# facebookresearch/VideoPose3D

Measured on NVIDIA H100. Metric: frames/sec (arc 3,3,3,3,3, T=243, N=1024), higher is better.
Workload: dtype fp16 (IEEE fp16 operands and activations, fp32 accumulate)

## Files before the change

videopose3d_b200/csrc/api.cu:

```cuda
#include <cuda.h>
#include <cuda_runtime.h>
#include <stdarg.h>
#include <stdio.h>
#include <stdlib.h>
#include <string.h>

#include <string>
#include <vector>

#include "internal.cuh"
#include "pack.cuh"
#include "train_ops.cuh"

using namespace vp3d;

static thread_local char g_err[512] = "";
namespace vp3d {
int fail(int code, const char* fmt, ...) {
  va_list ap;
  va_start(ap, fmt);
  vsnprintf(g_err, sizeof(g_err), fmt, ap);
  va_end(ap);
  return code;
}
// ... 57 lines not shown
                   box, estr, CU_TENSOR_MAP_INTERLEAVE_NONE, CU_TENSOR_MAP_SWIZZLE_128B,
                   CU_TENSOR_MAP_L2_PROMOTION_L2_256B, CU_TENSOR_MAP_FLOAT_OOB_FILL_NONE);
  if (r != CUDA_SUCCESS)
    return fail(VP3D_ERR_CUDA, "cuTensorMapEncodeTiled(2d) failed: %d (inner=%llu rows=%llu)",
                (int)r, (unsigned long long)inner, (unsigned long long)rows);
  return VP3D_OK;
}

int pick_block_n(int n_pad) {
  if (n_pad % 128 == 0) return 128;
  return 64;
}

static int g_sm_limit = 0;
int num_sms() {
  static int cache[kMaxDevices] = {};
  int dev = 0;
  if (cudaGetDevice(&dev) != cudaSuccess || dev < 0 || dev >= kMaxDevices) return 132;
  if (!cache[dev]) {
    int n = 0;
    cudaDeviceGetAttribute(&n, cudaDevAttrMultiProcessorCount, dev);
    cache[dev] = n > 0 ? n : 132;
    if (const char* e = getenv("VP3D_SM_LIMIT")) {
      const int lim = atoi(e);
      if (lim >= 2 && !g_sm_limit) g_sm_limit = lim;
    }
  }
  int n = cache[dev];
  if (g_sm_limit >= 2 && g_sm_limit < n) n = g_sm_limit;
  return n;
}

struct ConvLaunch {
  CUtensorMap ma, mw, mo, mr, mz;
  ConvGemmArgs g;
  int block_n = 64;
  int sms = 0;
  bool empty = false;
};

static int prepare_conv(const vp3d_conv_desc* d, ConvLaunch* L) {
  if (!d || !d->a || !d->w) return fail(VP3D_ERR_INVALID, "conv_gemm: null operand");
  if (d->a_ld % 64 || d->k_per_tap % 64 || d->n_pad % 64)
    return fail(VP3D_ERR_INVALID, "conv_gemm: a_ld, k_per_tap and n_pad must be multiples of 64");
  if (d->taps < 1 || d->out_rows < 0 || d->samples < 1)
    return fail(VP3D_ERR_INVALID, "conv_gemm: bad geometry");
  L->empty = d->out_rows == 0;
  if (L->empty) return VP3D_OK;
  const int a_planes = d->a_planes > 0 ? d->a_planes : 1;
  const int pairs = d->precision == VP3D_PRECISION_BF16X3 ? 3 : 1;
  const int i8 = d->precision == VP3D_PRECISION_INT8 ? 1 : 0;
  const int f16 = (d->precision == VP3D_PRECISION_FP16 || i8) ? 1 : 0;
  if (f16 && (a_planes != 1 || d->out_planes > 1 || d->stats || d->bnb_z))
    return fail(VP3D_ERR_INVALID, "conv_gemm: fp16 is a single-plane, inference-only format");
  if (i8 && (d->k_per_tap % kBlockK8 || d->tap_col_step != 0))
    return fail(VP3D_ERR_INVALID, "conv_gemm: int8 needs k_per_tap %% 128 == 0 and taps that step "
                "rows (tap_col_step 0)");
  if (d->out_u8 && (!f16 || d->out_u8_ld % 16 || d->out_u8_ld < d->n_pad ||
                    reinterpret_cast<uintptr_t>(d->out_u8) % 16))
    return fail(VP3D_ERR_INVALID, "conv_gemm: a u8 output needs fp16 or int8, a 16-byte aligned "
                "pointer and out_u8_ld >= n_pad, a multiple of 16");
  if ((i8 || d->out_u8) &&
      (!d->scale || !d->shift || !d->relu || d->out_f32 || d->res_col_begin || d->res_cols ||
       (d->res && d->res_planes > 1) || (i8 && d->res && !d->out) ||
       (i8 && !d->res && (d->out || !d->out_u8)) || (!i8 && (!d->out || d->res))))
    return fail(VP3D_ERR_UNSUPPORTED, "conv_gemm: int8 and u8 outputs exist for affine + ReLU "
                "[+ one-plane residual over every column] launches: int8 writes u8 alone or, with a "
// ... 110 lines not shown
      g.res_tma_col_off = (int)col_off;
      g.res_tma_row_off = (int)row_off;
    }
  }
  CUtensorMap& mz = L->mz;
  mz = mo;
  g.bnb = 0;
  if (d->bnb_z) {
    if (!d->out || g.out_planes != 1 || (d->res && !g.res_tma) || d->bnb_c <= 0 || d->bnb_c % 64)
      return fail(VP3D_ERR_INVALID, "conv_gemm: fused BN-backward needs a single-plane bf16 output, "
                  "a TMA-loadable residual (if any) and bnb_c % 64 == 0");
    const uint64_t o_rows = d->out_rows, o_ld = d->out_ld;
    const uint64_t o_samples = d->per_sample_tiles ? d->samples : 1;
    VP3D_TRY(make_map_4d(&mz, d->bnb_z, o_ld, o_rows, o_ld, o_samples, o_rows * o_ld, 1,
                         o_samples * o_rows * o_ld, kBlockM));
    g.bnb = 1;
    g.bnb_c = d->bnb_c;
    g.bnb_scale = d->bnb_scale; g.bnb_shift = d->bnb_shift; g.bnb_mean = d->bnb_mean;
    g.bnb_invstd = d->bnb_invstd; g.bnb_sums = d->bnb_sums;
    g.bnb_p = d->bnb_p;
    g.bnb_seed_lo = (unsigned)(d->bnb_seed & 0xFFFFFFFFu);
    g.bnb_seed_hi = (unsigned)(d->bnb_seed >> 32);
    g.bnb_layer = (unsigned)d->bnb_layer;
  }
  if (d->out_u8) {
    const uint64_t rows = d->out_rows, ld = d->out_u8_ld;
    const uint64_t smp = d->per_sample_tiles ? d->samples : 1;
    VP3D_TRY(make_map_4d(&mz, d->out_u8, d->n_pad, rows, ld, smp, rows * ld, 1, smp * rows * ld, 32,
                         1, 64, CU_TENSOR_MAP_SWIZZLE_NONE));
  }
  if ((i8 || d->out_u8) && d->res && !g.res_tma)
    return fail(VP3D_ERR_UNSUPPORTED, "conv_gemm: int8 / u8-output launches need a residual that "
                "TMA can load (one box of a strided row view)");
  VP3D_TRY(make_map_2d(&mw, d->w, d->k_per_tap, (uint64_t)w_planes * d->taps * d->n_pad, block_n,
                       i8 ? 1 : 2));
  return VP3D_OK;
}

int run_conv(const vp3d_conv_desc* d, cudaStream_t stream) {
  ConvLaunch L;
  VP3D_TRY(prepare_conv(d, &L));
  if (L.empty) return VP3D_OK;
  CUDA_TRY(launch_conv_gemm(L.ma, L.mw, L.mo, L.mr, L.mz, L.g, L.block_n, L.sms, stream));
  return VP3D_OK;
}

static int conv_instance(const vp3d_conv_desc* d, int* key) {
  if (!key) return fail(VP3D_ERR_INVALID, "conv_gemm_instance: null key");
  ConvLaunch L;
  VP3D_TRY(prepare_conv(d, &L));
  if (L.empty) return fail(VP3D_ERR_INVALID, "conv_gemm_instance: no output rows, nothing is launched");
  if (!conv_gemm_instance(L.g, L.block_n, L.sms, key))
    return fail(VP3D_ERR_UNSUPPORTED, "conv_gemm_instance: the selected instance is not compiled");
  return VP3D_OK;
}

int plan_alloc(vp3d_plan* p, void** out, size_t bytes) {
  void* q = nullptr;
  CUDA_TRY(cudaMalloc(&q, bytes));
  p->allocs.push_back(q);
  *out = q;
  return VP3D_OK;
}

static int conv_k_pad(const vp3d_plan* p, int l) {
  return block_is_int8(p, l / 2 + 1) ? round_up(p->C, kBlockK8) : p->C;
}

static size_t pack_capacity(const vp3d_plan* p, const PackedConv& k) {
  const size_t b = pack_bytes(p, k);
  if (!p->int8 || k.transposed || k.src < 0) return b;
  const size_t b16 = (size_t)k.stored_taps * k.n_pad * p->C * sizeof(__nv_bfloat16);
  return b > b16 ? b : b16;
}

static void plan_packs(vp3d_plan* p) {
// ... 907 lines not shown
```

videopose3d_b200/csrc/conv_gemm.cu:

```cuda
#include "conv_gemm.cuh"

#include <stdlib.h>
#include <string.h>

#include <type_traits>

#include "ptx.cuh"

namespace vp3d {

enum class Epi { kTrain, kGeneral, kLean };
enum class Fmt { kRuntime, kBf16, kF16, kI8 };
enum class Sched { kCooperative, kPingPong };
enum class U8Out { kNone, kBeside, kAlone };

struct InstKey {
  int block_n;
  Epi epi;
  Fmt fmt;
  Sched sched;
  bool res;
  bool out2;
  U8Out u8;
  constexpr bool operator==(const InstKey& o) const {
// ... 35 lines not shown
  static constexpr uint32_t kHalfBytes = 64 * 64 * 2;
  static constexpr uint32_t kStagingBytes =
      kPP ? (RES ? 0 : 2 * kTileBytes) : 2 * 2 * (OUT2 ? 2 : 1) * kHalfBytes;
  static constexpr int kResSlots = RES ? 4 : 0;
  static constexpr uint32_t kU8Bytes = kU8Beside ? 2 * kBlockM * 64 : 0;
  static constexpr uint32_t kFixedBytes = kStagingBytes + kResSlots * kTileBytes + kU8Bytes;
  static constexpr uint32_t kAffineBytes = kPP ? 0 : 2 * BLOCK_N * 4;
  static constexpr uint32_t kPairBytes = kTrain ? 4 * 2 * 64 * 4 : 0;
  static constexpr uint32_t kBarBytesMax = (2 * 8 + 8 + 1) * 8 + 32;
  static constexpr uint32_t kMaxSmem = 232448u;
  static constexpr int kStagesFit =
      (kMaxSmem - 1024 - kFixedBytes - kBarBytesMax - kAffineBytes - kPairBytes) / kStageBytes;
  static constexpr int kStages = kStagesFit > 8 ? 8 : kStagesFit;
  static_assert(kStages >= 2, "not enough shared memory for the operand pipeline");
  static constexpr uint32_t kBarBytes = (2 * kStages + 8 + 1) * 8 + 32;
  static constexpr uint32_t kSmemBytes =
      1024 + kStages * kStageBytes + kFixedBytes + kBarBytes + kAffineBytes + kPairBytes;
  static_assert(kSmemBytes <= kMaxSmem, "shared memory budget exceeded");
};

__device__ __forceinline__ void tile_coords(const ConvGemmArgs& p, int tile, int& n_blk,
                                            int& sample, int& row0) {
  n_blk = tile % p.n_tiles;
  int m_blk = tile / p.n_tiles;
  if (p.dilated) {
    sample = m_blk / p.tiles_per_sample;
    row0 = (m_blk - sample * p.tiles_per_sample) * kBlockM;
  } else {
    sample = 0;
    row0 = m_blk * kBlockM;
  }
}

__device__ __forceinline__ uint32_t ld_shared_u32(uint32_t addr) {
  uint32_t v;
  asm volatile("ld.shared.b32 %0, [%1];" : "=r"(v) : "r"(addr) : "memory");
  return v;
}
__device__ __forceinline__ void st_shared_u32(uint32_t addr, uint32_t v) {
  asm volatile("st.shared.b32 [%0], %1;" ::"r"(addr), "r"(v) : "memory");
}
__device__ __forceinline__ uint32_t sw128_off(int row, int c) {
  return (uint32_t)row * 128u + ((((uint32_t)c >> 3) ^ ((uint32_t)row & 7u)) << 4) + ((uint32_t)c & 7u) * 2u;
}
__device__ __forceinline__ void add_pair(float& a, float& b, uint32_t u, bool f16) {
  if (f16) { a += f16_lo_to_f(u); b += f16_hi_to_f(u); }
  else { a += bf16_lo_to_f(u); b += bf16_hi_to_f(u); }
}

__device__ __forceinline__ void st_u8_pair(uint32_t addr, float v0, float v1, float inv_s) {
  const uint32_t q = quant_u8(v0, inv_s) | (quant_u8(v1, inv_s) << 8);
  asm volatile("st.shared.u16 [%0], %1;" ::"r"(addr), "h"((unsigned short)q) : "memory");
}

__device__ __forceinline__ void slab_reduce(float (&s)[8][2], float (&q)[8][2], float* s_pair,
                                            int lane, int wq, uint32_t bar_id) {
#pragma unroll
  for (int off = 4; off <= 16; off <<= 1) {
#pragma unroll
    for (int jj = 0; jj < 8; ++jj) {
#pragma unroll
      for (int e = 0; e < 2; ++e) {
        s[jj][e] += __shfl_xor_sync(0xffffffffu, s[jj][e], off);
        q[jj][e] += __shfl_xor_sync(0xffffffffu, q[jj][e], off);
      }
    }
// ... 5 lines not shown
      *reinterpret_cast<float2*>(s_pair + 64 + 8 * jj + 2 * lane) = make_float2(q[jj][0], q[jj][1]);
    }
  }
  named_bar_sync(bar_id, 64);
  if (!(wq & 1) && lane < 4) {
#pragma unroll
    for (int jj = 0; jj < 8; ++jj) {
      const float2 so = *reinterpret_cast<const float2*>(s_pair + 8 * jj + 2 * lane);
      const float2 qo = *reinterpret_cast<const float2*>(s_pair + 64 + 8 * jj + 2 * lane);
      s[jj][0] += so.x; s[jj][1] += so.y;
      q[jj][0] += qo.x; q[jj][1] += qo.y;
    }
  }
  named_bar_sync(bar_id, 64);
}

#ifdef VP3D_TIMELINE
__device__ __forceinline__ void tl_stamp(const ConvGemmArgs& p, int ev) {
  if (!p.timeline) return;
  int slot;
  if (blockIdx.x == 0) slot = 0;
  else if (blockIdx.x == gridDim.x - 1) slot = 1;
  else return;
  unsigned long long g;
  asm volatile("mov.u64 %0, %%globaltimer;" : "=l"(g));
  p.timeline[(slot * 32 + ev) * 2] = g;
  p.timeline[(slot * 32 + ev) * 2 + 1] = (unsigned long long)clock64();
}
#define TL(ev) tl_stamp(p, ev)
#else
#define TL(ev) ((void)0)
#endif

template <int BLOCK_N, Fmt FMT, int H, class Acc>
__device__ __forceinline__ void wgmma_kblock(Acc (&acc)[H][BLOCK_N / 2], const uint64_t (&da)[H],
                                             uint64_t db, bool first) {
#pragma unroll
  for (int h = 0; h < H; ++h) {
#pragma unroll
    for (int k = 0; k < 4; ++k) {
      const uint32_t accumulate = (first && k == 0) ? 0u : 1u;
      if constexpr (FMT == Fmt::kI8) {
        if constexpr (BLOCK_N == 128) wgmma_m64n128k32_u8s8(acc[h], da[h] + 2 * k, db + 2 * k, accumulate);
        else wgmma_m64n64k32_u8s8(acc[h], da[h] + 2 * k, db + 2 * k, accumulate);
      } else if constexpr (BLOCK_N == 128) {
        if constexpr (FMT == Fmt::kF16) wgmma_m64n128_f16(acc[h], da[h] + 2 * k, db + 2 * k, accumulate);
        else wgmma_m64n128_bf16(acc[h], da[h] + 2 * k, db + 2 * k, accumulate);
      } else {
        if constexpr (FMT == Fmt::kF16) wgmma_m64n64_f16(acc[h], da[h] + 2 * k, db + 2 * k, accumulate);
        else wgmma_m64n64_bf16(acc[h], da[h] + 2 * k, db + 2 * k, accumulate);
      }
    }
  }
}

template <class I, int H, class Issued>
__device__ __forceinline__ void mma_tile(typename I::Acc (&acc)[H][I::kBlockN / 2],
                                         const ConvGemmArgs& p, bool f16, uint32_t smem_a,
                                         uint32_t a_off, uint32_t smem_b, uint32_t full_bar,
                                         uint32_t empty_bar, uint32_t& stage_io, uint32_t& phase_io,
                                         int k_iters, int lane, bool tl_first, Issued issued) {
  uint32_t stage = stage_io, phase = phase_io;
  uint32_t prev_stage = 0;
  for (int it = 0; it < k_iters; ++it) {
    mbar_wait(full_bar + stage * 8, phase);
#ifdef VP3D_TIMELINE
    if (tl_first && it == 0) TL(4);
#endif
    const uint32_t a_st = smem_a + stage * I::kABytes + a_off;
    uint64_t da[H];
#pragma unroll
    for (int h = 0; h < H; ++h) da[h] = make_gmma_desc_sw128(a_st + h * 64 * 128, 16, 1024);
    const uint64_t db = make_gmma_desc_sw128(smem_b + stage * I::kBBytes, 16, 1024);
#pragma unroll
    for (int h = 0; h < H; ++h) wgmma_fence_operands(acc[h]);
    wgmma_fence();
    if constexpr (I::kFmt != Fmt::kRuntime) wgmma_kblock<I::kBlockN, I::kFmt>(acc, da, db, it == 0);
    else if (f16) wgmma_kblock<I::kBlockN, Fmt::kF16>(acc, da, db, it == 0);
    else wgmma_kblock<I::kBlockN, Fmt::kBf16>(acc, da, db, it == 0);
    wgmma_commit();
#pragma unroll
    for (int h = 0; h < H; ++h) wgmma_fence_operands(acc[h]);
    if (it > 0) {
      wgmma_wait<1>();
#pragma unroll
      for (int h = 0; h < H; ++h) wgmma_fence_operands(acc[h]);
      if (lane == 0) mbar_arrive(empty_bar + prev_stage * 8);
    }
    prev_stage = stage;
    if (++stage == I::kStages) { stage = 0; phase ^= 1; }
  }
  stage_io = stage; phase_io = phase;
  issued();
  wgmma_wait<0>();
#pragma unroll
  for (int h = 0; h < H; ++h) wgmma_fence_operands(acc[h]);
  if (k_iters > 0 && lane == 0) mbar_arrive(empty_bar + prev_stage * 8);
}

template <class I>
__global__ void __launch_bounds__(384, 1)
conv_gemm_kernel(const __grid_constant__ CUtensorMap tmap_a,
                 const __grid_constant__ CUtensorMap tmap_w,
                 const __grid_constant__ CUtensorMap tmap_out,
                 const __grid_constant__ CUtensorMap tmap_res,
                 const __grid_constant__ CUtensorMap tmap_z, const ConvGemmArgs p) {
  using Acc = typename I::Acc;
  constexpr int kBlocksPerTile = I::kBlockN / 64;
  constexpr int kFrag = I::kBlockN / 2;
  constexpr int kBK = I::kI8 ? kBlockK8 : kBlockK;

  extern __shared__ uint8_t smem_raw[];
  const uint32_t raw_addr = smem_u32(smem_raw);
  const uint32_t base = (raw_addr + 1023u) & ~1023u;
  uint8_t* smem = smem_raw + (base - raw_addr);

  const uint32_t smem_a = base;
  const uint32_t smem_b = base + I::kStages * I::kABytes;
  const uint32_t smem_store = base + I::kStages * I::kStageBytes;
  const uint32_t smem_res = smem_store + I::kStagingBytes;
  const uint32_t smem_u8 = smem_res + I::kResSlots * I::kTileBytes;
  const uint32_t bar_base = smem_u8 + I::kU8Bytes;
  const uint32_t full_bar = bar_base;
  const uint32_t empty_bar = bar_base + I::kStages * 8;
  const uint32_t rfull_bar = bar_base + 2 * I::kStages * 8;
  const uint32_t rempty_bar = rfull_bar + 32;
  const uint32_t dep_bar = rempty_bar + 32;
  const uint32_t affine_off = (dep_bar + 8 - base + 15u) & ~15u;
  float* s_affine = reinterpret_cast<float*>(smem + affine_off);
  float* s_pairs = reinterpret_cast<float*>(smem + affine_off + I::kAffineBytes);

  const int warp = threadIdx.x >> 5;
  const int lane = threadIdx.x & 31;
  if (threadIdx.x == 0) TL(0);

  const int m_tiles = p.dilated ? p.samples * p.tiles_per_sample : p.tiles_per_sample;
  const int total_tiles = m_tiles * p.n_tiles;
  const int k_iters = p.pairs * p.taps * p.kblocks_per_tap;
  const bool has_res = (p.flags & kEpiResidual) != 0;
  const bool bnb = I::kTrain && p.bnb != 0;
  const int aux_tiles = (has_res ? p.res_planes : 0) + (bnb ? 1 : 0);
  const int res_stages =
      (aux_tiles > 0 && I::kResSlots >= aux_tiles) ? I::kResSlots / aux_tiles : 1;

  if (warp == 0 && lane == 0) {
    tma_prefetch_desc(&tmap_a);
    tma_prefetch_desc(&tmap_w);
    tma_prefetch_desc(&tmap_out);
    if (I::kRes) tma_prefetch_desc(&tmap_res);
    if (I::kRes && bnb) tma_prefetch_desc(&tmap_z);
    if (I::kU8) tma_prefetch_desc(&tmap_z);
  }
  if (warp == 1 && lane == 0) {
    for (int s = 0; s < I::kStages; ++s) {
      mbar_init(full_bar + s * 8, 1);
      mbar_init(empty_bar + s * 8, I::kPP ? 4 : 8);
    }
    for (int s = 0; s < 4; ++s) {
      mbar_init(rfull_bar + s * 8, 1);
      mbar_init(rempty_bar + s * 8, I::kPP ? 1 : 256);
    }
    mbar_init(dep_bar, 1);
    fence_mbar_init();
  }
  __syncthreads();
  if (threadIdx.x == 0) TL(1);
  if (warp != 0) {
    griddep_wait();
    griddep_launch_dependents();
  }
  if (threadIdx.x == 32) {
    mbar_arrive(dep_bar);
    TL(2);
  }

  if (warp == 0) {
    if (lane == 0) {
      constexpr bool kEarlyW = !I::kTrain;
      if (!kEarlyW) mbar_wait(dep_bar, 0);
      const int n_pre = kEarlyW ? (k_iters < I::kStages ? k_iters : I::kStages) : 0;
      int mode = n_pre > 0 ? 0 : 2;
      if (kEarlyW && mode == 2) mbar_wait(dep_bar, 0);
      int w = blockIdx.x;
      if (w < total_tiles) {
        int n_blk, sample, row0;
        tile_coords(p, w, n_blk, sample, row0);
        uint32_t stage = 0, phase = 0;
        int it = 0, pair = 0, tap = 0, kb = 0;
        for (;;) {
          const int a_plane = (pair == 1) ? 1 : 0;
          const int w_plane = (pair == 2) ? 1 : 0;
          const uint32_t fb = full_bar + stage * 8;
          if (mode != 1) {
            mbar_wait(empty_bar + stage * 8, phase ^ 1);
            mbar_expect_tx(fb, I::kStageBytes);
            const int w_row = (w_plane * p.taps + tap) * p.n_pad + n_blk * I::kBlockN;
            tma_load_2d(&tmap_w, fb, smem_b + stage * I::kBBytes, kb * kBK, w_row);
          }
          if (mode != 0) {
            const int a_row = row0 + tap * p.tap_row_step;
            const int a_col = tap * p.tap_col_step + kb * kBK;
            tma_load_4d(&tmap_a, fb, smem_a + stage * I::kABytes, a_col, a_row, sample, a_plane);
#ifdef VP3D_TIMELINE
            if (w == (int)blockIdx.x && it == 0) TL(3);
#endif
          }
          if (++stage == I::kStages) { stage = 0; phase ^= 1; }
          ++it;
          if (++kb == p.kblocks_per_tap) {
            kb = 0;
            if (++tap == p.taps) { tap = 0; ++pair; }
          }
          if (mode == 0 && it == n_pre) {
            mbar_wait(dep_bar, 0);
            mode = 1;
            it = 0; pair = 0; tap = 0; kb = 0;
            stage = 0; phase = 0;
          } else if (mode == 1 && it == n_pre) {
            mode = 2;
          }
          if (it == k_iters) {
            w += gridDim.x;
            if (w >= total_tiles) break;
            tile_coords(p, w, n_blk, sample, row0);
            it = 0; pair = 0; tap = 0; kb = 0;
          }
        }
      }
    }
  } else if (warp == 1) {
    if (I::kPP && I::kRes && lane == 0) {
      uint32_t filled[2] = {0u, 0u};
      for (int j = 0, w = blockIdx.x; w < total_tiles; ++j, w += gridDim.x) {
        int n_blk, sample, row0;
        tile_coords(p, w, n_blk, sample, row0);
        const int g = j & 1;
        for (int sb = 0; sb < kBlocksPerTile; ++sb) {
          const uint32_t n = g ? filled[1] : filled[0];
          const uint32_t slot = 2u * g + (n & 1u);
          mbar_wait(rempty_bar + slot * 8, ((n >> 1) & 1u) ^ 1u);
          mbar_expect_tx(rfull_bar + slot * 8, I::kTileBytes);
          tma_load_4d(&tmap_res, rfull_bar + slot * 8, smem_res + slot * I::kTileBytes,
                      n_blk * I::kBlockN + sb * 64 + p.res_tma_col_off, row0 + p.res_tma_row_off,
                      sample, 0);
          if (g) ++filled[1];
          else ++filled[0];
        }
      }
    } else if (!I::kPP && I::kRes && lane == 0) {
      uint32_t rs = 0, rphase = 0;
      for (int w = blockIdx.x; w < total_tiles; w += gridDim.x) {
        int n_blk, sample, row0;
        tile_coords(p, w, n_blk, sample, row0);
        for (int sb = 0; sb < kBlocksPerTile; ++sb) {
          const int col = n_blk * I::kBlockN + sb * 64;
          const bool res_here = has_res && col >= p.res_col_begin && col < p.res_col_begin + p.res_cols;
          if (!res_here && !bnb) continue;
          const int n_res = res_here ? p.res_planes : 0;
          mbar_wait(rempty_bar + rs * 8, rphase ^ 1);
          mbar_expect_tx(rfull_bar + rs * 8, (n_res + (bnb ? 1 : 0)) * I::kTileBytes);
          const uint32_t slot0 = smem_res + rs * aux_tiles * I::kTileBytes;
          for (int pl = 0; pl < n_res; ++pl)
            tma_load_4d(&tmap_res, rfull_bar + rs * 8, slot0 + pl * I::kTileBytes,
                        col - p.res_col_begin + p.res_tma_col_off, row0 + p.res_tma_row_off, sample,
                        pl);
          if (bnb)
            tma_load_4d(&tmap_z, rfull_bar + rs * 8, slot0 + (aux_tiles - 1) * I::kTileBytes, col,
                        row0, sample, 0);
          if (++rs == (uint32_t)res_stages) { rs = 0; rphase ^= 1; }
        }
      }
    }
  } else if (I::kPP && warp >= 4) {
    const int wg = (warp - 4) >> 2;
    const int wq = warp & 3;
    const int tid = (int)threadIdx.x - 128 - 128 * wg;
    const int rl0 = 16 * wq + (lane >> 2);
    const int cq = 2 * (lane & 3);
    const uint32_t bar_wg = 2u + (uint32_t)wg;
    const uint32_t bar_mine = 8u + (uint32_t)wg, bar_other = 9u - (uint32_t)wg;
    const uint32_t staging = smem_store + wg * I::kTileBytes;
    uint32_t res_seen = 0;
    Acc acc[2][kFrag];
#pragma unroll
    for (int i = 0; i < kFrag; ++i) acc[0][i] = acc[1][i] = 0.0f;

    for (int j = wg, w = blockIdx.x + wg * gridDim.x; w < total_tiles; j += 2, w += 2 * gridDim.x) {
      int n_blk, sample, row0;
      tile_coords(p, w, n_blk, sample, row0);

      const uint32_t fill = (uint32_t)j * (uint32_t)k_iters;
      uint32_t stage = fill % I::kStages, phase = (fill / I::kStages) & 1u;
      if (j > 0) named_bar_sync(bar_mine, 256);
      mma_tile<I>(acc, p, I::kF16, smem_a, 0u, smem_b, full_bar, empty_bar, stage, phase, k_iters,
                  lane, warp == 4 && lane == 0 && w == (int)blockIdx.x, [&] {
                    if (w + (int)gridDim.x < total_tiles) named_bar_arrive(bar_other, 256);
                  });
#ifdef VP3D_TIMELINE
      if (warp == 4 && lane == 0) { if (w == (int)blockIdx.x) TL(7); TL(8); }
#endif

      const float* scale = p.scale + n_blk * I::kBlockN;
      const float* shift = p.shift + n_blk * I::kBlockN;
#pragma unroll
      for (int sb = 0; sb < kBlocksPerTile; ++sb) {
        const int cb = n_blk * I::kBlockN + sb * 64;
        uint32_t tile_smem;
        if constexpr (I::kRes) {
          const uint32_t slot = 2u * wg + (res_seen & 1u);
          mbar_wait(rfull_bar + slot * 8, (res_seen >> 1) & 1u);
          ++res_seen;
          tile_smem = smem_res + slot * I::kTileBytes;
          if constexpr (I::kU8) {
            if (tid == 0) tma_store_wait_read<0>();
            named_bar_sync(bar_wg, 128);
          }
        } else {
          if (tid == 0) tma_store_wait_read<0>();
          named_bar_sync(bar_wg, 128);
          tile_smem = staging;
        }
        const uint32_t u8_tile = I::kU8Alone ? staging : smem_u8 + (uint32_t)wg * (kBlockM * 64);
#pragma unroll
        for (int jj = 0; jj < 8; ++jj) {
          const int j4 = 4 * (sb * 8 + jj);
          const int cl = sb * 64 + jj * 8 + cq;
          const float2 sc = __ldg(reinterpret_cast<const float2*>(scale + cl));
          const float2 sh = __ldg(reinterpret_cast<const float2*>(shift + cl));
#pragma unroll
          for (int h2 = 0; h2 < 2; ++h2) {
#pragma unroll
            for (int h = 0; h < 2; ++h) {
              float v0 = fmaxf(fmaf(static_cast<float>(acc[h2][j4 + 2 * h]), sc.x, sh.x), 0.0f);
              float v1 = fmaxf(fmaf(static_cast<float>(acc[h2][j4 + 2 * h + 1]), sc.y, sh.y), 0.0f);
              const uint32_t off = sw128_off(64 * h2 + rl0 + 8 * h, jj * 8 + cq);
              if (I::kRes) add_pair(v0, v1, ld_shared_u32(tile_smem + off), I::kF16);
              if constexpr (I::kStore16)
                st_shared_u32(tile_smem + off, I::kF16 ? pack_f16x2(v0, v1) : pack_bf16x2(v0, v1));
              if constexpr (I::kU8)
                st_u8_pair(u8_tile + (uint32_t)(64 * h2 + rl0 + 8 * h) * 64u + jj * 8 + cq, v0, v1,
                           p.u8_inv_s);
            }
          }
        }
        fence_proxy_async_smem();
        named_bar_sync(bar_wg, 128);
        if (tid == 0) {
#pragma unroll
          for (int hb = 0; hb < 4; ++hb) {
            if constexpr (I::kStore16)
              tma_store_4d(&tmap_out, tile_smem + hb * 4096u, cb, row0 + 32 * hb, sample, 0);
            if constexpr (I::kU8)
              tma_store_4d(&tmap_z, u8_tile + hb * 2048u, cb, row0 + 32 * hb, sample, 0);
          }
          tma_store_commit();
        }
      }
      if (I::kRes && tid == 0) {
        tma_store_wait_read<0>();
#pragma unroll
        for (int sb = 0; sb < kBlocksPerTile; ++sb)
          mbar_arrive(rempty_bar + (2u * wg + ((res_seen - kBlocksPerTile + sb) & 1u)) * 8);
      }
#ifdef VP3D_TIMELINE
      if (warp == 4 && lane == 0) { if (w == (int)blockIdx.x) TL(9); TL(10); }
#endif
    }
    if (tid == 0) tma_store_wait_all<0>();
#ifdef VP3D_TIMELINE
    if (warp == 4 && lane == 0) TL(11);
#endif
  } else if (!I::kPP && warp >= 4) {
    const int wg = (warp - 4) >> 2;
    const int wq = warp & 3;
    const int tid = (int)threadIdx.x - 128 - 128 * wg;
    const int rl0 = 16 * wq + (lane >> 2);
    const int cq = 2 * (lane & 3);
    const uint32_t bar_wg = 2u + (uint32_t)wg;
    const uint32_t bar_slab = 4u + (uint32_t)(wg * 2 + (wq >> 1));
    float* s_pair = s_pairs + (wg * 2 + (wq >> 1)) * 128;
    const bool f16 = I::kLean ? I::kF16 : p.f16 != 0;
    const bool do_relu = I::kLean || (p.flags & kEpiRelu);
    const bool do_res = I::kLean ? I::kRes : (p.flags & kEpiResidual) != 0;
    const bool do_stats = I::kTrain && (p.flags & kEpiStats);
    const bool do_f32 = !I::kLean && (p.flags & kEpiOutF32);
    const bool do_affine = I::kLean || (p.flags & kEpiAffine);
    const bool two_planes = I::kOut2 && p.out_planes == 2;
    uint32_t stage = 0, phase = 0;
    uint32_t ablock = 0;
    uint32_t sbuf = 0;
    int aff_n_blk = -1;
    Acc acc[1][kFrag];
#pragma unroll
    for (int i = 0; i < kFrag; ++i) acc[0][i] = 0.0f;

    for (int w = blockIdx.x; w < total_tiles; w += gridDim.x) {
      int n_blk, sample, row0;
      tile_coords(p, w, n_blk, sample, row0);
      const int m_blk = w / p.n_tiles;
// ... 203 lines not shown
          }
          sbuf ^= 1u;
        }
      }
#ifdef VP3D_TIMELINE
      if (warp == 4 && lane == 0) { if (w == (int)blockIdx.x) TL(9); TL(10); }
#endif
    }
    if (tid == 0) tma_store_wait_all<0>();
#ifdef VP3D_TIMELINE
    if (warp == 4 && lane == 0) TL(11);
#endif
  }
}

static int g_pdl = -1;
static bool pdl_enabled() {
  if (g_pdl < 0) {
    const char* e = getenv("VP3D_PDL");
    g_pdl = (e && e[0] == '0') ? 0 : 1;
  }
  return g_pdl != 0;
}
void conv_gemm_set_pdl(int on) { g_pdl = on ? 1 : 0; }
bool conv_gemm_pdl_enabled() { return pdl_enabled(); }

static int conv_tiles(const ConvGemmArgs& a) {
  const int m_tiles = a.dilated ? a.samples * a.tiles_per_sample : a.tiles_per_sample;
  return m_tiles * a.n_tiles;
}

template <class I>
static cudaError_t launch_impl(const CUtensorMap& tmap_a, const CUtensorMap& tmap_w,
                               const CUtensorMap& tmap_out, const CUtensorMap& tmap_res,
                               const CUtensorMap& tmap_z, const ConvGemmArgs& args, int num_sms,
                               cudaStream_t stream) {
  auto kernel = conv_gemm_kernel<I>;
  static bool attr_set[kMaxDevices] = {};
  int dev = 0;
  cudaError_t e = cudaGetDevice(&dev);
  if (e != cudaSuccess) return e;
  if (dev < 0 || dev >= kMaxDevices) return cudaErrorInvalidDevice;
  if (!attr_set[dev]) {
    e = cudaFuncSetAttribute(kernel, cudaFuncAttributeMaxDynamicSharedMemorySize, I::kSmemBytes);
    if (e != cudaSuccess) return e;
    attr_set[dev] = true;
  }
  const int total = conv_tiles(args);
  if (total <= 0) return cudaSuccess;
  const int workers = total < num_sms ? total : num_sms;
  cudaLaunchConfig_t cfg;
  memset(&cfg, 0, sizeof(cfg));
  cfg.gridDim = dim3(workers, 1, 1);
  cfg.blockDim = dim3(384, 1, 1);
  cfg.dynamicSmemBytes = I::kSmemBytes;
  cfg.stream = stream;
  cudaLaunchAttribute attr[1];
  int n_attr = 0;
  if (pdl_enabled()) {
    attr[n_attr].id = cudaLaunchAttributeProgrammaticStreamSerialization;
    attr[n_attr].val.programmaticStreamSerializationAllowed = 1;
    ++n_attr;
  }
  cfg.attrs = attr;
  cfg.numAttrs = n_attr;
  return cudaLaunchKernelEx(&cfg, kernel, tmap_a, tmap_w, tmap_out, tmap_res, tmap_z, args);
}

static bool lean_enabled() {
  static int v = -1;
  if (v < 0) {
    const char* e = getenv("VP3D_LEAN");
    v = (e && e[0] == '0') ? 0 : 1;
  }
  return v != 0;
}
static bool lean_ok(const ConvGemmArgs& a, bool res) {
  if (!lean_enabled() || a.bnb || a.out_planes != 1 || !a.out) return false;
  if (!res) return a.flags == (kEpiAffine | kEpiRelu) && !a.res_tma;
  return a.flags == (kEpiAffine | kEpiRelu | kEpiResidual) && a.res_tma && a.res_planes == 1 &&
         a.res_col_begin == 0 && a.res_cols >= a.n_pad;
}

static InstKey select_instance(const ConvGemmArgs& a, int block_n, bool multi_tile) {
  InstKey k = {block_n, Epi::kGeneral, Fmt::kRuntime, Sched::kCooperative, a.res_tma || a.bnb,
               a.out_planes == 2 && !(a.flags & kEpiOutF32), U8Out::kNone};
  if ((a.flags & kEpiStats) || a.bnb) {
    k.epi = Epi::kTrain;
    return k;
  }
  const bool quant = a.i8 || a.out_u8;
  if (!quant && (k.out2 || !lean_ok(a, k.res))) return k;
  k.epi = Epi::kLean;
  k.fmt = a.i8 ? Fmt::kI8 : a.f16 ? Fmt::kF16 : Fmt::kBf16;
  if (a.out_u8) k.u8 = a.out ? U8Out::kBeside : U8Out::kAlone;
  if (multi_tile) k.sched = Sched::kPingPong;
  return k;
}

template <class... Is>
struct InstList {};

template <int BN>
using Instances = InstList<
    Inst<BN, Epi::kTrain, Fmt::kRuntime, Sched::kCooperative, false, false>,
    Inst<BN, Epi::kTrain, Fmt::kRuntime, Sched::kCooperative, false, true>,
    Inst<BN, Epi::kTrain, Fmt::kRuntime, Sched::kCooperative, true, false>,
    Inst<BN, Epi::kTrain, Fmt::kRuntime, Sched::kCooperative, true, true>,
    Inst<BN, Epi::kGeneral, Fmt::kRuntime, Sched::kCooperative, false, false>,
    Inst<BN, Epi::kGeneral, Fmt::kRuntime, Sched::kCooperative, false, true>,
    Inst<BN, Epi::kGeneral, Fmt::kRuntime, Sched::kCooperative, true, false>,
    Inst<BN, Epi::kGeneral, Fmt::kRuntime, Sched::kCooperative, true, true>,
    Inst<BN, Epi::kLean, Fmt::kBf16, Sched::kCooperative, false>,
    Inst<BN, Epi::kLean, Fmt::kBf16, Sched::kCooperative, true>,
    Inst<BN, Epi::kLean, Fmt::kBf16, Sched::kPingPong, false>,
    Inst<BN, Epi::kLean, Fmt::kBf16, Sched::kPingPong, true>,
    Inst<BN, Epi::kLean, Fmt::kF16, Sched::kCooperative, false>,
    Inst<BN, Epi::kLean, Fmt::kF16, Sched::kCooperative, true>,
    Inst<BN, Epi::kLean, Fmt::kF16, Sched::kPingPong, false>,
    Inst<BN, Epi::kLean, Fmt::kF16, Sched::kPingPong, true>,
    Inst<BN, Epi::kLean, Fmt::kI8, Sched::kCooperative, false, false, U8Out::kAlone>,
    Inst<BN, Epi::kLean, Fmt::kI8, Sched::kCooperative, true, false, U8Out::kNone>,
    Inst<BN, Epi::kLean, Fmt::kI8, Sched::kCooperative, true, false, U8Out::kBeside>,
    Inst<BN, Epi::kLean, Fmt::kF16, Sched::kCooperative, false, false, U8Out::kBeside>,
    Inst<BN, Epi::kLean, Fmt::kI8, Sched::kPingPong, false, false, U8Out::kAlone>,
    Inst<BN, Epi::kLean, Fmt::kI8, Sched::kPingPong, true, false, U8Out::kNone>,
    Inst<BN, Epi::kLean, Fmt::kI8, Sched::kPingPong, true, false, U8Out::kBeside>,
    Inst<BN, Epi::kLean, Fmt::kF16, Sched::kPingPong, false, false, U8Out::kBeside>>;

template <class... Is>
static cudaError_t launch_listed(InstList<Is...>, const InstKey& k, const CUtensorMap& a,
                                 const CUtensorMap& w, const CUtensorMap& o, const CUtensorMap& r,
                                 const CUtensorMap& z, const ConvGemmArgs& args, int num_sms,
                                 cudaStream_t stream) {
  cudaError_t e = cudaErrorInvalidValue;
  (void)((k == Is::kKey && ((e = launch_impl<Is>(a, w, o, r, z, args, num_sms, stream)), true)) ||
         ...);
  return e;
}

#ifdef VP3D_TIMELINE
static unsigned long long* g_timeline = nullptr;
static int g_timeline_max = 0, g_timeline_next = 0;
void conv_gemm_debug_set_timeline(unsigned long long* buf, int max_launches) {
  g_timeline = buf;
  g_timeline_max = max_launches;
  g_timeline_next = 0;
}
#endif

static InstKey launch_key(const ConvGemmArgs& args, int block_n, int num_sms) {
  return select_instance(args, block_n, conv_tiles(args) > num_sms);
}

template <class... Is>
static bool listed(InstList<Is...>, const InstKey& k) {
  return ((k == Is::kKey) || ...);
}

static void key_ints(const InstKey& k, int* out) {
  out[0] = k.block_n;
  out[1] = (int)k.epi;
  out[2] = (int)k.fmt;
  out[3] = (int)k.sched;
  out[4] = k.res ? 1 : 0;
  out[5] = k.out2 ? 1 : 0;
  out[6] = (int)k.u8;
}

bool conv_gemm_instance(const ConvGemmArgs& args, int block_n, int num_sms, int key[7]) {
  const InstKey k = launch_key(args, block_n, num_sms);
  key_ints(k, key);
  return block_n == 128 ? listed(Instances<128>{}, k) : listed(Instances<64>{}, k);
}

template <class... Is>
static int list_keys(InstList<Is...>, int* keys, int max) {
  const InstKey all[] = {Is::kKey...};
  const int n = (int)sizeof...(Is);
  for (int i = 0; i < n && i < max; ++i) key_ints(all[i], keys + 7 * i);
  return n;
}

int conv_gemm_instances(int* keys, int max) {
  const int n128 = list_keys(Instances<128>{}, keys, max);
  const int done = n128 < max ? n128 : max;
  return n128 + list_keys(Instances<64>{}, keys + 7 * done, max - done);
}

cudaError_t launch_conv_gemm(const CUtensorMap& tmap_a, const CUtensorMap& tmap_w,
                             const CUtensorMap& tmap_out, const CUtensorMap& tmap_res,
                             const CUtensorMap& tmap_z, const ConvGemmArgs& args_in, int block_n,
                             int num_sms, cudaStream_t stream) {
#ifdef VP3D_TIMELINE
  ConvGemmArgs args = args_in;
  args.timeline = (g_timeline && g_timeline_next < g_timeline_max)
                      ? g_timeline + (size_t)(g_timeline_next++) * 128 : nullptr;
#else
  const ConvGemmArgs& args = args_in;
#endif
  const InstKey k = launch_key(args, block_n, num_sms);
  if (block_n == 128)
    return launch_listed(Instances<128>{}, k, tmap_a, tmap_w, tmap_out, tmap_res, tmap_z, args, num_sms, stream);
  return launch_listed(Instances<64>{}, k, tmap_a, tmap_w, tmap_out, tmap_res, tmap_z, args, num_sms, stream);
}

}
```

videopose3d_b200/csrc/conv_gemm.cuh:

```cuda
#pragma once
#include <cuda.h>
#include <cuda_bf16.h>
#include <cuda_runtime.h>
#include <stdint.h>

namespace vp3d {

constexpr int kBlockM = 128;
constexpr int kBlockK = 64;
constexpr int kBlockK8 = 128;
constexpr int kUmmaK = 16;
constexpr int kMaxDevices = 64;

enum ConvGemmFlags : int {
  kEpiRelu = 1,
  kEpiResidual = 2,
  kEpiStats = 4,
  kEpiOutF32 = 8,
  kEpiAffine = 16,
};

struct ConvGemmArgs {
  int dilated;
  int samples;
// ... 15 lines not shown
  int res_planes;
  int res_ld;
  int res_rows_per_sample;
  int res_row_step;
  int res_row_off;
  int res_sample_div;
  int res_col_begin;
  int res_cols;
  int res_check_rows;
  int res_tma;
  int res_tma_col_off;
  int res_tma_row_off;
  int bnb;
  int bnb_c;
  const float* bnb_scale;
  const float* bnb_shift;
  const float* bnb_mean;
  const float* bnb_invstd;
  float* bnb_sums;
  float bnb_p;
  unsigned bnb_seed_lo, bnb_seed_hi, bnb_layer;
  __nv_bfloat16* out;
  long long out_plane_stride;
  int out_planes;
  int out_ld;
  float* out_f32;
  int out_f32_ld;
  int n_valid;
  float* stats;
  int lo_row_begin, lo_row_end;
  int i8;
  uint8_t* out_u8;
  float u8_inv_s;
#ifdef VP3D_TIMELINE
  unsigned long long* timeline;
#endif
};
#ifdef VP3D_TIMELINE
void conv_gemm_debug_set_timeline(unsigned long long* buf, int max_launches);
#endif

void conv_gemm_set_pdl(int on);
bool conv_gemm_pdl_enabled();
bool conv_gemm_instance(const ConvGemmArgs& args, int block_n, int num_sms, int key[7]);
int conv_gemm_instances(int* keys, int max);
cudaError_t launch_conv_gemm(const CUtensorMap& tmap_a, const CUtensorMap& tmap_w,
                             const CUtensorMap& tmap_out, const CUtensorMap& tmap_res,
                             const CUtensorMap& tmap_z, const ConvGemmArgs& args, int block_n,
                             int num_sms, cudaStream_t stream);

}
```

Measured before the change: 1.411 million.

## Split tail-wave 128-wide tiles into 64-wide halves in ping-pong conv GEMM

For ping-pong instances with 128-column tiles, the leftover tiles that would form a partial last wave are each split into two 64-column half items. These are spread across more CTAs using a separate 64-row weight tensor map and n64 wgmma. The aim is to shrink the wave-quantization tail, where only a few SMs are busy on the final tiles. The cost is extra A-tile loads for each half item and more complex producer, residual and epilogue bookkeeping.

```diff
diff --git a/videopose3d_b200/csrc/api.cu b/videopose3d_b200/csrc/api.cu
--- a/videopose3d_b200/csrc/api.cu
+++ b/videopose3d_b200/csrc/api.cu
@@ -113,7 +113,7 @@
 }
 
 struct ConvLaunch {
-  CUtensorMap ma, mw, mo, mr, mz;
+  CUtensorMap ma, mw, mw64, mo, mr, mz;
   ConvGemmArgs g;
   int block_n = 64;
   int sms = 0;
@@ -290,8 +290,10 @@
   if ((i8 || d->out_u8) && d->res && !g.res_tma)
     return fail(VP3D_ERR_UNSUPPORTED, "conv_gemm: int8 / u8-output launches need a residual that "
                 "TMA can load (one box of a strided row view)");
-  VP3D_TRY(make_map_2d(&mw, d->w, d->k_per_tap, (uint64_t)w_planes * d->taps * d->n_pad, block_n,
-                       i8 ? 1 : 2));
+  const uint64_t w_rows = (uint64_t)w_planes * d->taps * d->n_pad;
+  VP3D_TRY(make_map_2d(&mw, d->w, d->k_per_tap, w_rows, block_n, i8 ? 1 : 2));
+  L->mw64 = mw;
+  if (block_n == 128) VP3D_TRY(make_map_2d(&L->mw64, d->w, d->k_per_tap, w_rows, 64, i8 ? 1 : 2));
   return VP3D_OK;
 }
 
@@ -299,7 +301,7 @@
   ConvLaunch L;
   VP3D_TRY(prepare_conv(d, &L));
   if (L.empty) return VP3D_OK;
-  CUDA_TRY(launch_conv_gemm(L.ma, L.mw, L.mo, L.mr, L.mz, L.g, L.block_n, L.sms, stream));
+  CUDA_TRY(launch_conv_gemm(L.ma, L.mw, L.mw64, L.mo, L.mr, L.mz, L.g, L.block_n, L.sms, stream));
   return VP3D_OK;
 }
 
diff --git a/videopose3d_b200/csrc/conv_gemm.cu b/videopose3d_b200/csrc/conv_gemm.cu
--- a/videopose3d_b200/csrc/conv_gemm.cu
+++ b/videopose3d_b200/csrc/conv_gemm.cu
@@ -91,6 +91,14 @@
   }
 }
 
+__device__ __forceinline__ bool item_coords(const ConvGemmArgs& p, int full_tiles, int w,
+                                            int& n_blk, int& sample, int& row0, int& c_off) {
+  const bool half = w >= full_tiles;
+  c_off = half ? 64 * ((w - full_tiles) & 1) : 0;
+  tile_coords(p, half ? full_tiles + ((w - full_tiles) >> 1) : w, n_blk, sample, row0);
+  return half;
+}
+
 __device__ __forceinline__ uint32_t ld_shared_u32(uint32_t addr) {
   uint32_t v;
   asm volatile("ld.shared.b32 %0, [%1];" : "=r"(v) : "r"(addr) : "memory");
@@ -162,29 +170,31 @@
 #define TL(ev) ((void)0)
 #endif
 
-template <int BLOCK_N, Fmt FMT, int H, class Acc>
-__device__ __forceinline__ void wgmma_kblock(Acc (&acc)[H][BLOCK_N / 2], const uint64_t (&da)[H],
+template <int N, Fmt FMT, int H, int F, class Acc>
+__device__ __forceinline__ void wgmma_kblock(Acc (&acc)[H][F], const uint64_t (&da)[H],
                                              uint64_t db, bool first) {
+  static_assert((N == 64 || N == 128) && N / 2 <= F, "not a wgmma width of this accumulator");
 #pragma unroll
   for (int h = 0; h < H; ++h) {
+    auto& d = reinterpret_cast<Acc(&)[N / 2]>(acc[h]);
 #pragma unroll
     for (int k = 0; k < 4; ++k) {
       const uint32_t accumulate = (first && k == 0) ? 0u : 1u;
       if constexpr (FMT == Fmt::kI8) {
-        if constexpr (BLOCK_N == 128) wgmma_m64n128k32_u8s8(acc[h], da[h] + 2 * k, db + 2 * k, accumulate);
-        else wgmma_m64n64k32_u8s8(acc[h], da[h] + 2 * k, db + 2 * k, accumulate);
-      } else if constexpr (BLOCK_N == 128) {
-        if constexpr (FMT == Fmt::kF16) wgmma_m64n128_f16(acc[h], da[h] + 2 * k, db + 2 * k, accumulate);
-        else wgmma_m64n128_bf16(acc[h], da[h] + 2 * k, db + 2 * k, accumulate);
+        if constexpr (N == 128) wgmma_m64n128k32_u8s8(d, da[h] + 2 * k, db + 2 * k, accumulate);
+        else wgmma_m64n64k32_u8s8(d, da[h] + 2 * k, db + 2 * k, accumulate);
+      } else if constexpr (N == 128) {
+        if constexpr (FMT == Fmt::kF16) wgmma_m64n128_f16(d, da[h] + 2 * k, db + 2 * k, accumulate);
+        else wgmma_m64n128_bf16(d, da[h] + 2 * k, db + 2 * k, accumulate);
       } else {
-        if constexpr (FMT == Fmt::kF16) wgmma_m64n64_f16(acc[h], da[h] + 2 * k, db + 2 * k, accumulate);
-        else wgmma_m64n64_bf16(acc[h], da[h] + 2 * k, db + 2 * k, accumulate);
+        if constexpr (FMT == Fmt::kF16) wgmma_m64n64_f16(d, da[h] + 2 * k, db + 2 * k, accumulate);
+        else wgmma_m64n64_bf16(d, da[h] + 2 * k, db + 2 * k, accumulate);
       }
     }
   }
 }
 
-template <class I, int H, class Issued>
+template <class I, int N = I::kBlockN, int H, class Issued>
 __device__ __forceinline__ void mma_tile(typename I::Acc (&acc)[H][I::kBlockN / 2],
                                          const ConvGemmArgs& p, bool f16, uint32_t smem_a,
                                          uint32_t a_off, uint32_t smem_b, uint32_t full_bar,
@@ -205,9 +215,9 @@
 #pragma unroll
     for (int h = 0; h < H; ++h) wgmma_fence_operands(acc[h]);
     wgmma_fence();
-    if constexpr (I::kFmt != Fmt::kRuntime) wgmma_kblock<I::kBlockN, I::kFmt>(acc, da, db, it == 0);
-    else if (f16) wgmma_kblock<I::kBlockN, Fmt::kF16>(acc, da, db, it == 0);
-    else wgmma_kblock<I::kBlockN, Fmt::kBf16>(acc, da, db, it == 0);
+    if constexpr (I::kFmt != Fmt::kRuntime) wgmma_kblock<N, I::kFmt>(acc, da, db, it == 0);
+    else if (f16) wgmma_kblock<N, Fmt::kF16>(acc, da, db, it == 0);
+    else wgmma_kblock<N, Fmt::kBf16>(acc, da, db, it == 0);
     wgmma_commit();
 #pragma unroll
     for (int h = 0; h < H; ++h) wgmma_fence_operands(acc[h]);
@@ -232,6 +242,7 @@
 __global__ void __launch_bounds__(384, 1)
 conv_gemm_kernel(const __grid_constant__ CUtensorMap tmap_a,
                  const __grid_constant__ CUtensorMap tmap_w,
+                 const __grid_constant__ CUtensorMap tmap_w64,
                  const __grid_constant__ CUtensorMap tmap_out,
                  const __grid_constant__ CUtensorMap tmap_res,
                  const __grid_constant__ CUtensorMap tmap_z, const ConvGemmArgs p) {
@@ -266,6 +277,10 @@
 
   const int m_tiles = p.dilated ? p.samples * p.tiles_per_sample : p.tiles_per_sample;
   const int total_tiles = m_tiles * p.n_tiles;
+  constexpr bool kHalves = I::kPP && I::kBlockN == 128;
+  const int half_items = kHalves ? p.half_items : 0;
+  const int full_tiles = total_tiles - half_items / 2;
+  const int n_items = full_tiles + half_items;
   const int k_iters = p.pairs * p.taps * p.kblocks_per_tap;
   const bool has_res = (p.flags & kEpiResidual) != 0;
   const bool bnb = I::kTrain && p.bnb != 0;
@@ -276,6 +291,7 @@
   if (warp == 0 && lane == 0) {
     tma_prefetch_desc(&tmap_a);
     tma_prefetch_desc(&tmap_w);
+    if (kHalves && half_items > 0) tma_prefetch_desc(&tmap_w64);
     tma_prefetch_desc(&tmap_out);
     if (I::kRes) tma_prefetch_desc(&tmap_res);
     if (I::kRes && bnb) tma_prefetch_desc(&tmap_z);
@@ -312,7 +328,7 @@
       int mode = n_pre > 0 ? 0 : 2;
       if (kEarlyW && mode == 2) mbar_wait(dep_bar, 0);
       int w = blockIdx.x;
-      if (w < total_tiles) {
+      if (w < full_tiles) {
         int n_blk, sample, row0;
         tile_coords(p, w, n_blk, sample, row0);
         uint32_t stage = 0, phase = 0;
@@ -351,9 +367,31 @@
           }
           if (it == k_iters) {
             w += gridDim.x;
-            if (w >= total_tiles) break;
+            if (w >= full_tiles) break;
             tile_coords(p, w, n_blk, sample, row0);
             it = 0; pair = 0; tap = 0; kb = 0;
+          }
+        }
+        if constexpr (kHalves) {
+          if (w < n_items) {
+            int c_off;
+            item_coords(p, full_tiles, w, n_blk, sample, row0, c_off);
+            for (int h_it = 0, h_pair = 0, h_tap = 0, h_kb = 0; h_it < k_iters; ++h_it) {
+              const uint32_t fb = full_bar + stage * 8;
+              mbar_wait(empty_bar + stage * 8, phase ^ 1);
+              mbar_expect_tx(fb, I::kABytes + I::kBBytes / 2);
+              const int w_row = ((h_pair == 2 ? 1 : 0) * p.taps + h_tap) * p.n_pad +
+                                n_blk * I::kBlockN + c_off;
+              tma_load_2d(&tmap_w64, fb, smem_b + stage * I::kBBytes, h_kb * kBK, w_row);
+              tma_load_4d(&tmap_a, fb, smem_a + stage * I::kABytes,
+                          h_tap * p.tap_col_step + h_kb * kBK, row0 + h_tap * p.tap_row_step,
+                          sample, h_pair == 1 ? 1 : 0);
+              if (++stage == I::kStages) { stage = 0; phase ^= 1; }
+              if (++h_kb == p.kblocks_per_tap) {
+                h_kb = 0;
+                if (++h_tap == p.taps) { h_tap = 0; ++h_pair; }
+              }
+            }
           }
         }
       }
@@ -361,17 +399,18 @@
   } else if (warp == 1) {
     if (I::kPP && I::kRes && lane == 0) {
       uint32_t filled[2] = {0u, 0u};
-      for (int j = 0, w = blockIdx.x; w < total_tiles; ++j, w += gridDim.x) {
-        int n_blk, sample, row0;
-        tile_coords(p, w, n_blk, sample, row0);
+      for (int j = 0, w = blockIdx.x; w < n_items; ++j, w += gridDim.x) {
+        int n_blk, sample, row0, c_off;
+        const bool half = item_coords(p, full_tiles, w, n_blk, sample, row0, c_off);
         const int g = j & 1;
-        for (int sb = 0; sb < kBlocksPerTile; ++sb) {
+        for (int sb = 0; sb < (half ? 1 : kBlocksPerTile); ++sb) {
           const uint32_t n = g ? filled[1] : filled[0];
           const uint32_t slot = 2u * g + (n & 1u);
           mbar_wait(rempty_bar + slot * 8, ((n >> 1) & 1u) ^ 1u);
           mbar_expect_tx(rfull_bar + slot * 8, I::kTileBytes);
           tma_load_4d(&tmap_res, rfull_bar + slot * 8, smem_res + slot * I::kTileBytes,
-                      n_blk * I::kBlockN + sb * 64 + p.res_tma_col_off, row0 + p.res_tma_row_off,
+                      n_blk * I::kBlockN + c_off + sb * 64 + p.res_tma_col_off,
+                      row0 + p.res_tma_row_off,
                       sample, 0);
           if (g) ++filled[1];
           else ++filled[0];
@@ -415,26 +454,30 @@
 #pragma unroll
     for (int i = 0; i < kFrag; ++i) acc[0][i] = acc[1][i] = 0.0f;
 
-    for (int j = wg, w = blockIdx.x + wg * gridDim.x; w < total_tiles; j += 2, w += 2 * gridDim.x) {
-      int n_blk, sample, row0;
-      tile_coords(p, w, n_blk, sample, row0);
+    const auto run_item = [&](int j, int w, auto half_tag) {
+      constexpr bool kHalf = decltype(half_tag)::value;
+      constexpr int kSb = kHalf ? 1 : kBlocksPerTile;
+      int n_blk, sample, row0, c_off = 0;
+      if constexpr (kHalf) item_coords(p, full_tiles, w, n_blk, sample, row0, c_off);
+      else tile_coords(p, w, n_blk, sample, row0);
 
       const uint32_t fill = (uint32_t)j * (uint32_t)k_iters;
       uint32_t stage = fill % I::kStages, phase = (fill / I::kStages) & 1u;
       if (j > 0) named_bar_sync(bar_mine, 256);
-      mma_tile<I>(acc, p, I::kF16, smem_a, 0u, smem_b, full_bar, empty_bar, stage, phase, k_iters,
-                  lane, warp == 4 && lane == 0 && w == (int)blockIdx.x, [&] {
-                    if (w + (int)gridDim.x < total_tiles) named_bar_arrive(bar_other, 256);
-                  });
+      mma_tile<I, kHalf ? 64 : I::kBlockN>(
+          acc, p, I::kF16, smem_a, 0u, smem_b, full_bar, empty_bar, stage, phase, k_iters, lane,
+          warp == 4 && lane == 0 && w == (int)blockIdx.x, [&] {
+            if (w + (int)gridDim.x < n_items) named_bar_arrive(bar_other, 256);
+          });
 #ifdef VP3D_TIMELINE
       if (warp == 4 && lane == 0) { if (w == (int)blockIdx.x) TL(7); TL(8); }
 #endif
 
-      const float* scale = p.scale + n_blk * I::kBlockN;
-      const float* shift = p.shift + n_blk * I::kBlockN;
-#pragma unroll
-      for (int sb = 0; sb < kBlocksPerTile; ++sb) {
-        const int cb = n_blk * I::kBlockN + sb * 64;
+      const float* scale = p.scale + n_blk * I::kBlockN + c_off;
+      const float* shift = p.shift + n_blk * I::kBlockN + c_off;
+#pragma unroll
+      for (int sb = 0; sb < kSb; ++sb) {
+        const int cb = n_blk * I::kBlockN + c_off + sb * 64;
         uint32_t tile_smem;
         if constexpr (I::kRes) {
           const uint32_t slot = 2u * wg + (res_seen & 1u);
@@ -489,12 +532,17 @@
       if (I::kRes && tid == 0) {
         tma_store_wait_read<0>();
 #pragma unroll
-        for (int sb = 0; sb < kBlocksPerTile; ++sb)
-          mbar_arrive(rempty_bar + (2u * wg + ((res_seen - kBlocksPerTile + sb) & 1u)) * 8);
+        for (int sb = 0; sb < kSb; ++sb)
+          mbar_arrive(rempty_bar + (2u * wg + ((res_seen - kSb + sb) & 1u)) * 8);
       }
 #ifdef VP3D_TIMELINE
       if (warp == 4 && lane == 0) { if (w == (int)blockIdx.x) TL(9); TL(10); }
 #endif
+    };
+    int j = wg, w = blockIdx.x + wg * gridDim.x;
+    for (; w < full_tiles; j += 2, w += 2 * gridDim.x) run_item(j, w, std::false_type{});
+    if constexpr (kHalves) {
+      if (w < n_items) run_item(j, w, std::true_type{});
     }
     if (tid == 0) tma_store_wait_all<0>();
 #ifdef VP3D_TIMELINE
@@ -764,9 +812,9 @@
 
 template <class I>
 static cudaError_t launch_impl(const CUtensorMap& tmap_a, const CUtensorMap& tmap_w,
-                               const CUtensorMap& tmap_out, const CUtensorMap& tmap_res,
-                               const CUtensorMap& tmap_z, const ConvGemmArgs& args, int num_sms,
-                               cudaStream_t stream) {
+                               const CUtensorMap& tmap_w64, const CUtensorMap& tmap_out,
+                               const CUtensorMap& tmap_res, const CUtensorMap& tmap_z,
+                               const ConvGemmArgs& args_in, int num_sms, cudaStream_t stream) {
   auto kernel = conv_gemm_kernel<I>;
   static bool attr_set[kMaxDevices] = {};
   int dev = 0;
@@ -778,9 +826,15 @@
     if (e != cudaSuccess) return e;
     attr_set[dev] = true;
   }
-  const int total = conv_tiles(args);
+  const int total = conv_tiles(args_in);
   if (total <= 0) return cudaSuccess;
   const int workers = total < num_sms ? total : num_sms;
+  ConvGemmArgs args = args_in;
+  args.half_items = 0;
+  if constexpr (I::kPP && I::kBlockN == 128) {
+    const int left = total % workers;
+    if (left > 0 && 2 * left <= workers) args.half_items = 2 * left;
+  }
   cudaLaunchConfig_t cfg;
   memset(&cfg, 0, sizeof(cfg));
   cfg.gridDim = dim3(workers, 1, 1);
@@ -796,7 +850,8 @@
   }
   cfg.attrs = attr;
   cfg.numAttrs = n_attr;
-  return cudaLaunchKernelEx(&cfg, kernel, tmap_a, tmap_w, tmap_out, tmap_res, tmap_z, args);
+  return cudaLaunchKernelEx(&cfg, kernel, tmap_a, tmap_w, tmap_w64, tmap_out, tmap_res, tmap_z,
+                            args);
 }
 
 static bool lean_enabled() {
@@ -862,11 +917,13 @@
 
 template <class... Is>
 static cudaError_t launch_listed(InstList<Is...>, const InstKey& k, const CUtensorMap& a,
-                                 const CUtensorMap& w, const CUtensorMap& o, const CUtensorMap& r,
+                                 const CUtensorMap& w, const CUtensorMap& w64,
+                                 const CUtensorMap& o, const CUtensorMap& r,
                                  const CUtensorMap& z, const ConvGemmArgs& args, int num_sms,
                                  cudaStream_t stream) {
   cudaError_t e = cudaErrorInvalidValue;
-  (void)((k == Is::kKey && ((e = launch_impl<Is>(a, w, o, r, z, args, num_sms, stream)), true)) ||
+  (void)((k == Is::kKey &&
+          ((e = launch_impl<Is>(a, w, w64, o, r, z, args, num_sms, stream)), true)) ||
          ...);
   return e;
 }
@@ -921,9 +978,10 @@
 }
 
 cudaError_t launch_conv_gemm(const CUtensorMap& tmap_a, const CUtensorMap& tmap_w,
-                             const CUtensorMap& tmap_out, const CUtensorMap& tmap_res,
-                             const CUtensorMap& tmap_z, const ConvGemmArgs& args_in, int block_n,
-                             int num_sms, cudaStream_t stream) {
+                             const CUtensorMap& tmap_w64, const CUtensorMap& tmap_out,
+                             const CUtensorMap& tmap_res, const CUtensorMap& tmap_z,
+                             const ConvGemmArgs& args_in, int block_n, int num_sms,
+                             cudaStream_t stream) {
 #ifdef VP3D_TIMELINE
   ConvGemmArgs args = args_in;
   args.timeline = (g_timeline && g_timeline_next < g_timeline_max)
@@ -933,8 +991,10 @@
 #endif
   const InstKey k = launch_key(args, block_n, num_sms);
   if (block_n == 128)
-    return launch_listed(Instances<128>{}, k, tmap_a, tmap_w, tmap_out, tmap_res, tmap_z, args, num_sms, stream);
-  return launch_listed(Instances<64>{}, k, tmap_a, tmap_w, tmap_out, tmap_res, tmap_z, args, num_sms, stream);
-}
-
-}
+    return launch_listed(Instances<128>{}, k, tmap_a, tmap_w, tmap_w64, tmap_out, tmap_res, tmap_z,
+                         args, num_sms, stream);
+  return launch_listed(Instances<64>{}, k, tmap_a, tmap_w, tmap_w64, tmap_out, tmap_res, tmap_z,
+                       args, num_sms, stream);
+}
+
+}
diff --git a/videopose3d_b200/csrc/conv_gemm.cuh b/videopose3d_b200/csrc/conv_gemm.cuh
--- a/videopose3d_b200/csrc/conv_gemm.cuh
+++ b/videopose3d_b200/csrc/conv_gemm.cuh
@@ -71,6 +71,7 @@
   int i8;
   uint8_t* out_u8;
   float u8_inv_s;
+  int half_items;
 #ifdef VP3D_TIMELINE
   unsigned long long* timeline;
 #endif
@@ -84,8 +85,9 @@
 bool conv_gemm_instance(const ConvGemmArgs& args, int block_n, int num_sms, int key[7]);
 int conv_gemm_instances(int* keys, int max);
 cudaError_t launch_conv_gemm(const CUtensorMap& tmap_a, const CUtensorMap& tmap_w,
-                             const CUtensorMap& tmap_out, const CUtensorMap& tmap_res,
-                             const CUtensorMap& tmap_z, const ConvGemmArgs& args, int block_n,
-                             int num_sms, cudaStream_t stream);
+                             const CUtensorMap& tmap_w64, const CUtensorMap& tmap_out,
+                             const CUtensorMap& tmap_res, const CUtensorMap& tmap_z,
+                             const ConvGemmArgs& args, int block_n, int num_sms,
+                             cudaStream_t stream);
 
 }
```

After: 1.459 million, median of 6. 1.03x the previous value.
